# lmfaber/karma

Hardware: AMD Instinct MI355X
Metric: contigs+reads/sec for k-mer vec + shared-read graph build; HBM GB/s vs roofline (higher is better)
Workload: dtype u32 keys / i64 counts / f64 div

## Files before the change

### __graft_entry__.py

```python

import os
import subprocess
import sys

REPO = os.path.dirname(os.path.abspath(__file__))


def build() -> None:
    jobs = str(min(16, os.cpu_count() or 4))
    subprocess.run(["make", "-C", os.path.join(REPO, "karma_amd", "csrc"), "-j", jobs], check=True)
    subprocess.run(["make", "-C", os.path.join(REPO, "karma_amd", "csrc"), "fake_rccl"], check=True)
    subprocess.run(["make", "-C", os.path.join(REPO, "oracle")], check=True)
    sys.path.insert(0, REPO)
    import karma_amd
    from karma_amd import _lib

    _lib.load()


def smoke() -> None:
    from collections import OrderedDict

    import numpy as np

    sys.path.insert(0, REPO)
    from karma_amd import engine
    from oracle import oracle

    blob, offs, key_len = engine.synth_contigs(5, 300, 50, 900, 64)
    seqs = OrderedDict((f">ctg{i}", bytes(blob[offs[i]:offs[i + 1]]).decode()) for i in range(300))
    prof, cols, _ = engine.kmer_profile(seqs, "5p6")
    oprof, ocols, _ = oracle.calc_kmer_profile(seqs, "5p6")
    assert cols == ocols, "column set differs from the oracle"
    assert np.array_equal(prof.view(np.uint64), oprof.view(np.uint64)), "profile differs from the oracle"

    rec = engine.synth_records(5, 300, 0, 20000, True)
    e = engine.graph_from_records(rec, 300)
    r = rec.astype(np.int64)
    starts = np.flatnonzero(np.r_[True, r[1:, 0] != r[:-1, 0]])
    o = oracle.graph_groups(np.r_[starts, len(r)], r[:, 1], None, None, 300, dedup=True)
    assert np.array_equal(e.a, o["a"]) and np.array_equal(e.b, o["b"]), "edge set differs from the oracle"
    assert np.array_equal(e.weight.view(np.uint64), o["weight"].view(np.uint64)), "weights differ from the oracle"
    ef = engine.graph_from_records(engine.flag_records(rec), 300, flagged=True)
    assert np.array_equal(ef.a, o["a"]) and np.array_equal(ef.b, o["b"]), "flagged edge set differs from the oracle"
    assert np.array_equal(ef.weight.view(np.uint64), o["weight"].view(np.uint64)), "flagged weights differ"
    print(f"smoke ok: profile {prof.shape}, {len(e.a)} edges (pairs and flagged records), bit-exact vs oracle")


if __name__ == "__main__":
    build()
    if len(sys.argv) > 1 and sys.argv[1] == "smoke":
        smoke()
```

### karma_amd/csrc/graph_sets.hip

```cpp

#include <algorithm>
#include <cstdlib>
#include <cstring>
#include <memory>
#include <type_traits>

#include "karma_internal.h"

using namespace karma;

namespace {

#include "graph_device.h"

typedef unsigned int u32x4 __attribute__((ext_vector_type(4)));

constexpr int kMaxB = 2048;
constexpr int kMaxBc = 512;
constexpr int kNarrowB = 512, kNarrowBc = 128;
constexpr int kCrSmax = 64;
constexpr int kCrPieces = 512;
constexpr int kCgShift = 18;
constexpr int kOneGroupB = 128;
constexpr int kAppendMinBc = 129;
// ... 1438 lines not shown
                    pre += nibble_sum(w[i] & ((1u << bs) - 1u));
                    mine = (w[i] >> bs) & 15u;
                }
            }
            *beg = c * (int64_t)seg_cap * (kBinQ / 8) + pre;
            *len = mine;
            list_back(c, bucket < 32 ? h2.x : h2.y);
        },
        add8, nullptr, slots);
    __syncthreads();
    uint32_t* const wt = reinterpret_cast<uint32_t*>(slots) + wave * 64;
    auto stream8 = [&](uint64_t m, uint32_t seg) {
        const int n = __popcll(m);
        wave_lds_order();
        if (in_mask(m)) wt[rank_below(m)] = seg;
        wave_lds_order();
        u32x4 v[8];
#pragma unroll
        for (int t = 0; t < 8; ++t) {
            const int j = 8 * t + (lane >> 3);
            if (8 * t < n && j < n) v[t] = *reinterpret_cast<const u32x4*>(segs + (int64_t)wt[j] * kBinQ + 8 * (lane & 7));
        }
#pragma unroll
        for (int t = 0; t < 8; ++t)
            if (8 * t < n && 8 * t + (lane >> 3) < n) add8(v[t]);
    };
    const uint8_t bb = (uint8_t)bucket;
    const uint32_t nl = nlist;
    const bool listed = nl <= list_cap;
    const int64_t n_items = listed ? (int64_t)nl : c_hi - c_lo;
    for (int64_t i0 = (int64_t)wave * 64; i0 < n_items; i0 += kCRT) {
        const int64_t i = i0 + lane;
        const int64_t c = i < n_items ? c_lo + (listed ? (int64_t)blist[i] : i) : c_hi;
        uint4 h1 = {0u, 0u, 0u, 0u}, h2 = {0u, 0u, 0u, 0u}, h3 = {0u, 0u, 0u, 0u};
        if (c < c_hi) {
            h2 = hdr[kBinHdr * c + 2];
            h1 = hdr[kBinHdr * c + 1];
            h3 = hdr[kBinHdr * c + 3];
        }
        const uint64_t bm = h2.x | (uint64_t)h2.y << 32;
        uint64_t mb = lanes((bm >> bucket) & 1ull);
        if (!mb) continue;
        const uint32_t nb = h1.w;
        const uint32_t d[4] = {h2.z, h2.w, h3.x, h3.y};
        uint32_t hit = 0;
#pragma unroll
        for (int k = 0; k < 16; ++k)
            hit |= (((d[k >> 2] >> (8 * (k & 3))) & 0xFFu) == bb && (uint32_t)k < nb) ? 1u << k : 0u;
        for (uint32_t base = 0;;) {
            for (;;) {
                const uint64_t mm = lanes(in_mask(mb) && hit != 0u);
                if (!mm) break;
                uint32_t sg = 0;
                if (hit) {
                    const uint32_t k = (uint32_t)__builtin_ctz(hit);
                    hit &= hit - 1u;
                    sg = (uint32_t)c * seg_cap + seg_cap - 1u - (base + k);
                }
                stream8(mm, sg);
            }
            base += 16;
            mb &= lanes(base < nb);
            if (!mb) break;
            if (in_mask(mb)) {
                const u32x4 q = *reinterpret_cast<const u32x4*>(dir + c * (int64_t)dir_cap + base);
                const uint32_t e[4] = {q.x, q.y, q.z, q.w};
#pragma unroll
                for (int k = 0; k < 16; ++k)
                    hit |= (((e[k >> 2] >> (8 * (k & 3))) & 0xFFu) == bb && base + k < nb) ? 1u << k : 0u;
            }
        }
    }
    __syncthreads();
    uint32_t* out = part_ch + (int64_t)blockIdx.x * hn;
    for (int i = threadIdx.x; i < hn; i += kCRT) out[i] = h[slot(i)];
}

constexpr int kRT = 1024;
constexpr int kBand = 8192;
constexpr int kHashR = 4096;
constexpr int kHashF = 8192;
constexpr int kFT = 512;
constexpr int kSlotCap = kBand + kHashF;

template <int CAP, int THREADS>
struct HTab {
    uint32_t* keys;
    uint32_t* vals;
    int* nuniq;
    __device__ void init() {
        for (int t = threadIdx.x; t < CAP; t += THREADS) {
            keys[t] = kEmpty;
            vals[t] = 0;
        }
        if (threadIdx.x == 0) *nuniq = 0;
    }
    __device__ __forceinline__ bool insert(uint32_t key, uint32_t c) {
        uint32_t h = hash32(key) & (CAP - 1);
        for (int probe = 0; probe < CAP; ++probe) {
            const uint32_t k = __hip_atomic_load(&keys[h], __ATOMIC_RELAXED, __HIP_MEMORY_SCOPE_WORKGROUP);
            if (k == key) {
                atomicAdd(&vals[h], c);
                return true;
            }
            if (k == kEmpty) {
                const uint32_t old = atomicCAS(&keys[h], kEmpty, key);
                if (old == kEmpty || old == key) {
                    if (old == kEmpty) atomicAdd(nuniq, 1);
                    atomicAdd(&vals[h], c);
                    return true;
                }
            }
            h = (h + 1) & (CAP - 1);
        }
        return false;
    }
    __device__ int compact(int* cnt) {
        if (threadIdx.x == 0) *cnt = 0;
        __syncthreads();
        uint32_t my_k[CAP / THREADS], my_v[CAP / THREADS];
#pragma unroll
        for (int u = 0; u < CAP / THREADS; ++u) {
            my_k[u] = keys[u * THREADS + threadIdx.x];
            my_v[u] = vals[u * THREADS + threadIdx.x];
        }
        __syncthreads();
#pragma unroll
        for (int u = 0; u < CAP / THREADS; ++u) {
            if (my_k[u] != kEmpty) {
                const int pos = atomicAdd(cnt, 1);
                keys[pos] = my_k[u];
                vals[pos] = my_v[u];
            }
        }
        __syncthreads();
        return *cnt;
    }
};

__global__ void __launch_bounds__(kRT) pair_reduce_kernel(const uint32_t* __restrict__ pent, RunDir dir,
                                                          int n_pg, int bw, int bbits, int dbits, int B,
                                                          uint32_t* __restrict__ part_band,
                                                          uint32_t* __restrict__ part_keys,
                                                          uint32_t* __restrict__ part_cnt, int* __restrict__ part_n,
                                                          uint8_t* __restrict__ overflow) {
    __shared__ uint32_t band[kBand];
    __shared__ uint32_t hkeys[kHashR];
    __shared__ uint32_t hvals[kHashR];
    __shared__ int nuniq, cnt, ovf;
    __shared__ int slots[kRT];
    HTab<kHashR, kRT> t{hkeys, hvals, &nuniq};
    const int bucket = blockIdx.x / n_pg, grp = blockIdx.x % n_pg;
    const int band_n = dbits >= 0 ? (1 << (bw + dbits)) : 0;
    const uint32_t D = dbits >= 0 ? (1u << dbits) : 0u;
    int64_t f_lo, f_hi;
    group_range(dir.n, n_pg, grp, &f_lo, &f_hi);
    const int64_t sl = blockIdx.x;
    if (f_lo >= f_hi) {
        if (threadIdx.x == 0) part_n[sl] = -1;
        return;
    }
    t.init();
    for (int i = threadIdx.x; i < band_n; i += kRT) band[i] = 0;
    if (threadIdx.x == 0) ovf = 0;
    __syncthreads();
    const uint32_t bmask = (1u << bbits) - 1u, abase = (uint32_t)bucket << bw;
    auto add = [&](uint32_t e) {
        if (e == kEmpty) return;
        const uint32_t al = e >> bbits, d = (e & bmask) - (abase + al);
        if (d < D)
            __hip_atomic_fetch_add(&band[(al << dbits) | d], 1u, __ATOMIC_RELAXED, __HIP_MEMORY_SCOPE_WORKGROUP);
        else if (!t.insert(e, 1u))
            ovf = 1;
    };
    stream_runs(
        reinterpret_cast<const u32x4*>(pent), f_lo, f_hi, kRT,
        [&](int64_t f, int64_t* beg, uint32_t* len) {
            const uint32_t* o = dir.off + f * (B + 1) + bucket;
            *beg = (dir.base[f] + o[0]) >> 2;
            *len = (o[1] - o[0]) >> 2;
        },
        [&](const u32x4 v) {
            add(v.x), add(v.y), add(v.z), add(v.w);
            if (nuniq > kHashR - kHashR / 8) ovf = 1;
        },
        &ovf, slots);
    __syncthreads();
    if (ovf) {
        if (threadIdx.x == 0) overflow[bucket] = 1;
        return;
    }
    uint32_t* pb = part_band + sl * (int64_t)kBand;
    for (int i = threadIdx.x; i < band_n; i += kRT) pb[i] = band[i];
    const int n = t.compact(&cnt);
    uint32_t* pk = part_keys + sl * (int64_t)kHashR;
    uint32_t* pc = part_cnt + sl * (int64_t)kHashR;
    for (int i = threadIdx.x; i < n; i += kRT) {
        pk[i] = hkeys[i];
        pc[i] = hvals[i];
    }
    if (threadIdx.x == 0) part_n[sl] = n;
}

__device__ __forceinline__ uint32_t code_count(const uint32_t* __restrict__ part_ch, int n_cg, int bwc, int gi) {
    const int bc = gi >> (bwc + 3), i = gi & ((8 << bwc) - 1);
    const int hn = 8 << bwc;
    uint32_t k = 0;
    for (int g = 0; g < n_cg; ++g) k += part_ch[((int64_t)bc * n_cg + g) * hn + i];
    return k;
}

constexpr int kMaxSplit = 65;
struct SplitArgs {
    int n;
    int64_t b[kMaxSplit];
    int64_t* out;
};

template <int HF>
__global__ void __launch_bounds__(kFT) final_kernel(
    int n_pg, int n_cg, int bw, int bbits, int dbits, int bwc, const uint32_t* __restrict__ part_band,
    const uint32_t* __restrict__ part_ch, const uint32_t* __restrict__ part_keys,
    const uint32_t* __restrict__ part_cnt, const int* __restrict__ part_n, uint64_t* __restrict__ out_keys,
    int64_t* __restrict__ out_counts, int64_t* __restrict__ out_n, uint8_t* __restrict__ overflow, SplitArgs split,
    uint64_t* __restrict__ lb, int64_t* __restrict__ out_off) {
    __shared__ uint32_t bsum[kBand];
    __shared__ uint32_t rowpos[(kBand >> 3) + 1];
    __shared__ uint32_t hkeys[HF];
    __shared__ uint32_t hvals[HF];
    __shared__ uint32_t wsum[kFT / 64];
    __shared__ int nuniq, cnt;
    __shared__ int64_t base;
    const int bucket = blockIdx.x;
    auto skip = [&]() {
        if (threadIdx.x < 64) {
            const int64_t o = lookback_offset(lb, bucket, 0, (int)threadIdx.x);
            if (threadIdx.x == 0) {
                out_off[bucket] = o;
                out_n[bucket] = 0;
                if (bucket == (int)gridDim.x - 1) out_off[bucket + 1] = o;
            }
        }
    };
    if (overflow[bucket]) {
        skip();
        return;
    }
    HTab<HF, kFT> t{hkeys, hvals, &nuniq};
    const int band_n = dbits >= 0 ? (1 << (bw + dbits)) : 0;
    constexpr bool one_list = HF == kHashR;
    if (!one_list) t.init();
    for (int i = threadIdx.x; i < band_n; i += kFT) {
        uint32_t v = 0;
        for (int gi = 0; gi < n_pg; ++gi) {
            const int64_t sl = (int64_t)bucket * n_pg + gi;
            if (part_n[sl] >= 0) v += part_band[sl * kBand + i];
        }
        bsum[i] = v;
    }
    __syncthreads();
    if (n_cg > 0) {
        const int hn = 8 << bwc;
        for (int m0l = (bucket > 0 ? -3 : 0) + (int)threadIdx.x; m0l < (1 << bw); m0l += kFT) {
            const int64_t gi = ((int64_t)bucket << (bw + 3)) + 8 * (int64_t)m0l;
            const uint4* src = reinterpret_cast<const uint4*>(part_ch + (gi >> (bwc + 3)) * n_cg * hn + (gi & (hn - 1)));
            uint32_t k[8] = {};
            for (int g = 0; g < n_cg; ++g) {
                const uint4 a = src[(int64_t)g * (hn >> 2)], b = src[(int64_t)g * (hn >> 2) + 1];
                k[0] += a.x, k[1] += a.y, k[2] += a.z, k[3] += a.w;
                k[4] += b.x, k[5] += b.y, k[6] += b.z, k[7] += b.w;
            }
#pragma unroll
            for (int i1 = 0; i1 < 4; ++i1) {
                if (m0l + i1 < 0 || m0l + i1 >= (1 << bw)) continue;
#pragma unroll
                for (int j1 = i1; j1 < 4; ++j1) {
                    uint32_t acc = 0;
#pragma unroll
                    for (int M = 0; M < 8; ++M) {
                        const uint32_t bits = 1u | (uint32_t)M << 1;
                        if ((bits >> i1 & 1u) && (bits >> j1 & 1u)) acc += k[M];
                    }
                    if (acc) atomicAdd(&bsum[(m0l + i1) << dbits | (j1 - i1)], acc);
                }
            }
        }
        __syncthreads();
    }
    int nh;
    if (one_list) {
        nh = max(0, part_n[bucket]);
        for (int i = threadIdx.x; i < nh; i += kFT) {
            hkeys[i] = part_keys[(int64_t)bucket * kHashR + i];
            hvals[i] = part_cnt[(int64_t)bucket * kHashR + i];
        }
        __syncthreads();
    } else {
        for (int gi = 0; gi < n_pg; ++gi) {
            const int64_t sl = (int64_t)bucket * n_pg + gi;
            const int n = part_n[sl];
            bool full = false;
            for (int i = threadIdx.x; i < n; i += kFT)
                full |= !t.insert(part_keys[sl * kHashR + i], part_cnt[sl * kHashR + i]);
            if (__syncthreads_or(full)) {
                if (threadIdx.x == 0) overflow[bucket] = 1;
                skip();
                return;
            }
        }
        nh = t.compact(&cnt);
    }
    int p2 = 1;
    while (p2 < nh) p2 <<= 1;
    for (int i = nh + threadIdx.x; i < p2; i += kFT) {
        hkeys[i] = kEmpty;
// ... 633 lines not shown
                        KARMA_LAUNCH(ctx, "graph_classify",
                                     (classify2_kernel<decltype(ap)::value, true, decltype(rl)::value,
                                                       decltype(bn)::value, decltype(fl)::value>),
                                     cg, kCW, 0, C, Bn);
                        return KARMA_OK;
                    });
                };
                return bin ? go(std::false_type{}, std::true_type{})
                           : append ? go(std::true_type{}, std::false_type{}) : go(std::false_type{}, std::false_type{});
            });
        };
        if (probe) {
            KARMA_LAUNCH(ctx, "relabel_probe", relabel_probe_kernel, 1, kRelabelProbes, 0, rec, A, (uint32_t)N,
                         counters + 3, reinterpret_cast<uint64_t*>(cb), (int64_t)(ctrl_words + 2 * n_pblk + B));
            C.skip = counters + 3;
        } else if (fresh_ext) {
            C.skip = counters + 3;
            C.vote = counters + 4;
        }
        KARMA_TRY(classify(0, n_chunks));
    }
    KARMA_TRY(mark(1));
    if (A == 0) {
        KARMA_HIP(hipMemsetAsync(n_codes.ptr, 0, n_chunks * 4, ctx->stream));
        KARMA_HIP(hipMemsetAsync(n_gen.ptr, 0, n_chunks * 4, ctx->stream));
        if (bin) KARMA_HIP(hipMemsetAsync(bhdr.ptr, 0, n_chunks * 16 * kBinHdr, ctx->stream));
    }
    const RunDir cdir{cf_base.ptr, cf_off.ptr, counters + 1, blk_items};
    pdir = RunDir{pf_base.ptr, pf_off.ptr, counters + 2, blk_items + n_pblk};
    hipStream_t const main_stream = ctx->stream;
    const bool fork = fork_on() && !opts.single_stream && !(ctx->timing && ctx->timing_only.empty());
    hipStream_t fork_s = main_stream;
    if (fork) {
        KARMA_TRY(ctx_fork(ctx, !opts.fork));
        fork_s = opts.fork ? opts.fork : ctx->fork_stream;
        KARMA_HIP(hipEventRecord(ctx->fork_a, main_stream));
        KARMA_HIP(hipStreamWaitEvent(fork_s, ctx->fork_a, 0));
    }
    {
        StreamScope on_fork(ctx, fork_s);
        KARMA_LAUNCH(ctx, "graph_general", general_kernel, general_grid(ctx, n_chunks), kGW, 0, rec, A, (uint32_t)N,
                     codes.ptr, n_gen.ptr, n_chunks, plist.ptr, pcap, n_pl.ptr, blk_items + n_pblk, lpb, flags,
                     relabeled ? (const uint32_t*)remap_map.ptr : nullptr, (const unsigned*)(counters + 3), chunk);
        if (wide_p)
            KARMA_LAUNCH(ctx, "graph_pair_partition", partition_kernel<PairStreamWide>, n_pblk, kPT, 0, plist.ptr,
                         pcap, n_pl.ptr, n_chunks, lpb, g, pent.ptr, pdir);
        else
            KARMA_LAUNCH(ctx, "graph_pair_partition", partition_kernel<PairStream>, n_pblk, kPT, 0, plist.ptr, pcap,
                         n_pl.ptr, n_chunks, lpb, g, pent.ptr, pdir);
        KARMA_LAUNCH(ctx, "graph_pair_reduce", pair_reduce_kernel, nsl, kRT, 0, pent.ptr, pdir, n_pg, g.bw, g.bbits,
                     g.dbits, B, part_b.ptr, part_k.ptr, part_c.ptr, part_n.ptr, ovf);
        if (fork) KARMA_HIP(hipEventRecord(ctx->fork_b, fork_s));
    }
    if (bin) {
        KARMA_LAUNCH(ctx, "graph_code_reduce", code_seg_reduce_kernel, (int64_t)g.Bc * n_cg, kCRT, 0, bsegs.ptr,
                     reinterpret_cast<const uint4*>(bhdr.ptr), bdir.ptr, n_chunks, seg_cap, dir_cap, g.bwc, n_cg,
                     part_ch.ptr, back_list_cap(), slotted ? 1 : 0);
        KARMA_TRY(mark(2));
    } else if (g.Bc > 0) {
        uint16_t* const trash = cent.ptr + (ccap + 7) / 8 * 8;
        if (append && wide_c)
            KARMA_LAUNCH(ctx, "graph_code_partition", code_append_kernel<kMaxBc>, n_pblk, kPT, 0, codes.ptr, chunk,
                         n_codes.ptr, n_chunks, lpb, g, blk_hist.ptr, cent.ptr, trash, cdir, flags + 3);
        else if (append)
            KARMA_LAUNCH(ctx, "graph_code_partition", code_append_kernel<kNarrowBc>, n_pblk, kPT, 0, codes.ptr,
                         chunk, n_codes.ptr, n_chunks, lpb, g, blk_hist.ptr, cent.ptr, trash, cdir, flags + 3);
        else if (wide_c)
            KARMA_LAUNCH(ctx, "graph_code_partition", partition_kernel<CodeStreamWide>, n_pblk, kPT, 0, codes.ptr,
                         chunk, n_codes.ptr, n_chunks, lpb, g, cent.ptr, cdir);
        else
            KARMA_LAUNCH(ctx, "graph_code_partition", partition_kernel<CodeStream>, n_pblk, kPT, 0, codes.ptr, chunk,
                         n_codes.ptr, n_chunks, lpb, g, cent.ptr, cdir);
        KARMA_TRY(mark(2));
        KARMA_LAUNCH(ctx, "graph_code_reduce", code_reduce_kernel, (int64_t)g.Bc * n_cg, kCRT, 0, cent.ptr, cdir,
                     g.Bc, g.bwc, n_cg, part_ch.ptr);
    }
    KARMA_TRY(mark(4));
    if (fork) KARMA_HIP(hipStreamWaitEvent(main_stream, ctx->fork_b, 0));
    SplitArgs sa{};
    sa.n = (int)split_b.size();
    for (int r = 0; r < sa.n; ++r) sa.b[r] = split_b[r];
    sa.out = split_loc;
    if (n_pg == 1)
        KARMA_LAUNCH(ctx, "graph_bucket_final", final_kernel<kHashR>, B, kFT, 0, n_pg, n_cg, g.bw, g.bbits, g.dbits,
                     g.bwc, part_b.ptr, part_ch.ptr, part_k.ptr, part_c.ptr, part_n.ptr, slot_k.ptr, slot_c.ptr, n_per,
                     ovf, sa, lb, dst);
    else
        KARMA_LAUNCH(ctx, "graph_bucket_final", final_kernel<kHashF>, B, kFT, 0, n_pg, n_cg, g.bw, g.bbits, g.dbits,
                     g.bwc, part_b.ptr, part_ch.ptr, part_k.ptr, part_c.ptr, part_n.ptr, slot_k.ptr, slot_c.ptr, n_per,
                     ovf, sa, lb, dst);
    KARMA_TRY(mark(5));
    if (!deferred)
        KARMA_HIP(hipMemcpyAsync(const_cast<int64_t*>(hctrl), cb, ctrl_words * 8, hipMemcpyDeviceToHost,
                                 ctx->stream));
    return KARMA_OK;
}

int SetsJob::relabel() {
    const uint32_t n = (uint32_t)N;
    DevArray<uint32_t> rep, root;
    DevArray<unsigned> fill;
    DevArray<int64_t> size, base;
    KARMA_TRY(remap_map.alloc(ctx, N));
    KARMA_TRY(remap_inv.alloc(ctx, N));
    KARMA_TRY(rep.alloc(ctx, N));
    KARMA_TRY(root.alloc(ctx, N));
    KARMA_TRY(fill.alloc(ctx, N));
    KARMA_TRY(size.alloc(ctx, N + 1));
    KARMA_TRY(base.alloc(ctx, N + 1));
    KARMA_LAUNCH(ctx, "relabel_iota", iota_u32_kernel, grid_n(N), 256, 0, rep.ptr, N);
    const int64_t As = std::min<int64_t>(A, std::max<int64_t>(A / 32, int64_t(1) << 22));
    if (As) KARMA_LAUNCH(ctx, "relabel_hook", relabel_hook_kernel, grid_n(As), 256, 0, rec, As, n, rep.ptr);
    KARMA_HIP(hipMemsetAsync(size.ptr, 0, (N + 1) * 8, ctx->stream));
    KARMA_HIP(hipMemsetAsync(fill.ptr, 0, N * 4, ctx->stream));
    KARMA_LAUNCH(ctx, "relabel_root", relabel_root_kernel, grid_n(N + 1), 256, 0, rep.ptr, n, root.ptr, size.ptr);
    KARMA_TRY(scan_excl_i64(ctx, size.ptr, base.ptr, N + 1));
    KARMA_LAUNCH(ctx, "relabel_assign", relabel_assign_kernel, grid_n(N), 256, 0, root.ptr, base.ptr, n, fill.ptr,
                 remap_map.ptr, remap_inv.ptr);
    return KARMA_OK;
}

int SetsJob::finish(karma_pairs* out) {
    unsigned hc[4] = {0, 0, 0, 0};
    std::vector<uint8_t> hovf(B);
    int64_t U = 0;
    for (;;) {
        KARMA_HIP(hipStreamSynchronize(ctx->stream));
        const int* hf = reinterpret_cast<const int*>(hctrl);
        std::memcpy(hc, hctrl + 2, sizeof hc);
        std::memcpy(hovf.data(), hctrl + 6 + 2 * (B + 1), B);
        U = hctrl[6 + (B + 1) + B];
        KARMA_CHECK(!hf[0], KARMA_ERR_UNSORTED, "records are not grouped by read (read ids decrease)");
        KARMA_CHECK(!hf[1], KARMA_ERR_ARG, "a record's contig index is >= n_contigs (%lld)", (long long)N);
        KARMA_CHECK(!hf[3], KARMA_ERR_STATE, "code partition: block counts disagree with the classify histogram");
        if (!relabeled && hc[3]) {
            KARMA_TRY(relabel());
            relabeled = true;
            KARMA_TRY(launch());
            continue;
        }
        if (!hf[2]) break;
        KARMA_CHECK(attempt == 0, KARMA_ERR_STATE, "pair list capacity exceeded twice");
        attempt = 1;
        pcap = chunk * 9 / 2;
        KARMA_TRY(launch());
    }
    const unsigned n_big = hc[0];
    if (std::getenv("KARMA_DEBUG_GEN")) {
        std::vector<uint32_t> hg(n_chunks);
        KARMA_HIP(hipMemcpy(hg.data(), n_gen.ptr, n_chunks * 4, hipMemcpyDeviceToHost));
        uint64_t tot = 0;
        for (uint32_t x : hg) tot += x;
        std::fprintf(stderr, "[karma] general reads %llu, big reads %u, pair flushes %u\n", (unsigned long long)tot,
                     n_big, hc[2]);
    }
    DevArray<const uint64_t*> pk;
    DevArray<const int64_t*> pc;
    DevArray<int64_t> src_off;
    std::vector<std::unique_ptr<DevArray<uint64_t>>> keep_k;
    std::vector<std::unique_ptr<DevArray<int64_t>>> keep_c;
    const int64_t widen_threads = std::max<int64_t>(hc[2], (int64_t(8) << g.bw) + 24);
    bool any_ovf = false;
    for (int b = 0; b < B; ++b) {
        if (!hovf[b]) continue;
        if (!any_ovf) {
            KARMA_TRY(pk.alloc(ctx, B));
            KARMA_TRY(pc.alloc(ctx, B));
            KARMA_TRY(src_off.alloc(ctx, B));
            KARMA_HIP(hipMemcpyAsync(src_off.ptr, dst, B * 8, hipMemcpyDeviceToDevice, ctx->stream));
            KARMA_HIP(hipMemsetAsync(pk.ptr, 0, B * sizeof(void*), ctx->stream));
            KARMA_HIP(hipMemsetAsync(pc.ptr, 0, B * sizeof(void*), ctx->stream));
        }
        any_ovf = true;
// ... 152 lines not shown
```

### karma_amd/csrc/kmer.hip

```cpp

#include <algorithm>
#include <cstring>
#include <memory>

#include "karma_internal.h"

using namespace karma;

struct karma_contigs {
    karma_ctx* ctx = nullptr;
    int64_t n = 0, total = 0, words = 0, exc_bases = 0;
    int64_t zero_key_maxlen = -1;
    int64_t max_len = 0;
    DevArray<uint8_t> raw_own;
    DevArray<int64_t> off_own;
    DevArray<int32_t> keylen_own;
    const uint8_t* raw = nullptr;
    const int64_t* off = nullptr;
    const int32_t* keylen = nullptr;
    DevArray<int64_t> woff;
    DevArray<uint32_t> packed;
    DevArray<uint16_t> mask;
    DevArray<uint8_t> has_exc;
    DevArray<uint32_t> exc_list;
// ... 522 lines not shown
                }
            }
        }
        wave_lds_sync();
    }
}

template <bool C16>
__device__ __forceinline__ void write_row_wave(double* __restrict__ row, uint32_t* __restrict__ counts, int64_t M,
                                               int32_t klen, int* __restrict__ err, double* __restrict__ lut,
                                               int lane) {
    const double len = (double)klen;
    lut[lane] = lane ? (double)lane / len : 0.0;
    wave_lds_sync();
    auto val = [&](uint32_t a) {
        double v = lut[min(a, 63u)];
        if (a >= 64u) v = (double)a / len;
        return v;
    };
    if ((reinterpret_cast<uintptr_t>(row) & 15) == 0) {
        const int64_t M2 = M >> 1;
        for (int64_t j = lane; j < M2; j += 64) {
            uint32_t a, b;
            if (C16) {
                const uint32_t ab = counts[j];
                counts[j] = 0;
                a = ab & 0xFFFFu;
                b = ab >> 16;
            } else {
                const uint2 ab = reinterpret_cast<uint2*>(counts)[j];
                reinterpret_cast<uint2*>(counts)[j] = make_uint2(0u, 0u);
                a = ab.x;
                b = ab.y;
            }
            if ((a | b) && klen == 0) *err = 1;
            d2 v;
            v.x = val(a);
            v.y = val(b);
            typedef unsigned int u32x4_t __attribute__((ext_vector_type(4)));
            const uint64_t u = (uint64_t)row;
            const __amdgpu_buffer_rsrc_t rr = __builtin_amdgcn_make_buffer_rsrc(
                reinterpret_cast<void*>(((uint64_t)(uint32_t)__builtin_amdgcn_readfirstlane((int)(u >> 32)) << 32) |
                                        (uint32_t)__builtin_amdgcn_readfirstlane((int)(uint32_t)u)),
                0, (int)(M * 8), 0x00020000);
            const u32x4_t w = {(uint32_t)__double2loint(v.x), (uint32_t)__double2hiint(v.x),
                               (uint32_t)__double2loint(v.y), (uint32_t)__double2hiint(v.y)};
            __builtin_amdgcn_raw_buffer_store_b128(w, rr, (int)(j * 16), 0, kRowAux);
        }
        if ((M & 1) && lane == 0) {
            const uint32_t a = C16 ? counts[M >> 1] & 0xFFFFu : counts[M - 1];
            counts[C16 ? M >> 1 : M - 1] = 0;
            if (a && klen == 0) *err = 1;
            row_store(val(a), row + M - 1);
        }
    } else {
        uint16_t* c16 = reinterpret_cast<uint16_t*>(counts);
        for (int64_t j = lane; j < M; j += 64) {
            const uint32_t a = C16 ? c16[j] : counts[j];
            if (C16) c16[j] = 0;
            else counts[j] = 0;
            if (a && klen == 0) *err = 1;
            row_store(val(a), row + j);
        }
    }
}

__device__ __forceinline__ unsigned wave_total(unsigned x) {
    x += (unsigned)__builtin_amdgcn_update_dpp(0, (int)x, 0x111, 0xF, 0xF, false);
    x += (unsigned)__builtin_amdgcn_update_dpp(0, (int)x, 0x112, 0xF, 0xF, false);
    x += (unsigned)__builtin_amdgcn_update_dpp(0, (int)x, 0x114, 0xF, 0xF, false);
    x += (unsigned)__builtin_amdgcn_update_dpp(0, (int)x, 0x118, 0xF, 0xF, false);
    x += (unsigned)__builtin_amdgcn_update_dpp(0, (int)x, 0x142, 0xA, 0xF, false);
    x += (unsigned)__builtin_amdgcn_update_dpp(0, (int)x, 0x143, 0xC, 0xF, false);
    return (unsigned)__builtin_amdgcn_readlane((int)x, 63);
}

__host__ __device__ constexpr int64_t hist_words(int64_t M, bool c16) {
    return c16 ? (((M + 1) >> 1) + 3) & ~int64_t(3) : (M + 3) & ~int64_t(3);
}
__host__ __device__ constexpr int64_t tab_entries(bool p56, uint32_t S) { return p56 ? 1088 : (int64_t)S; }

constexpr int kProfWaves = 6;
template <bool P56, bool C16>
__global__ void __launch_bounds__(kPBlock) __attribute__((amdgpu_waves_per_eu(kProfWaves, kProfWaves)))
profile_wave_kernel(
    const uint32_t* __restrict__ packed, const uint16_t* __restrict__ mask, const uint8_t* __restrict__ has_exc,
    const int64_t* __restrict__ woff, const int64_t* __restrict__ off, const uint8_t* __restrict__ raw,
    const int32_t* __restrict__ keylen, int64_t n, int k, bool with_len, const int32_t* __restrict__ col_of_ord,
    const uint64_t* __restrict__ exc, int64_t X, const int32_t* __restrict__ col_of_exc, int64_t M,
    double* __restrict__ out, int64_t ld, int* __restrict__ err, int S, int64_t* __restrict__ row_tot,
    int64_t exc0, const int64_t* __restrict__ m_dev) {
    extern __shared__ __attribute__((aligned(16))) uint32_t lds[];
    const int wave = __builtin_amdgcn_readfirstlane(threadIdx.x >> 6), lane = threadIdx.x & 63, wpb = blockDim.x >> 6;
    uint16_t* tab = reinterpret_cast<uint16_t*>(lds);
    const int t_pad = (int)((tab_entries(P56, S) + 7) & ~7);
    const int h_words = (int)hist_words(M, C16);
    if (m_dev) {
        M = *m_dev;
        ld = M;
    }
    uint32_t* counts = lds + t_pad / 2 + wave * (h_words + kProfWin);
    uint32_t* win = counts + h_words;
    uint16_t* mbuf = reinterpret_cast<uint16_t*>(win + 80);
    double* lut = reinterpret_cast<double*>(win);
    if (P56) {
        for (int o = threadIdx.x; o < 1088; o += blockDim.x) {
            uint32_t ord;
            if (o < 1024) {
                ord = 5u * o;
            } else {
                const uint32_t h3 = o - 1024, c6 = h3 << 6 | rev3(h3);
                ord = (c6 >> 2) * 5u + 1u + (c6 & 3u);
            }
            tab[o] = (uint16_t)col_of_ord[ord];
        }
    } else {
        for (int o = threadIdx.x; o < S; o += blockDim.x) tab[o] = (uint16_t)col_of_ord[o];
    }
    for (int j = lane; j < h_words; j += 64) counts[j] = 0;
    __syncthreads();
    const int kmin = P56 ? 5 : k;
    struct Meta {
        int64_t s = 0, L = 0, w0 = 0;
        int32_t klen = 0;
        bool exc = false;
    };
    auto meta = [&](int64_t cc, Meta& m) {
        if (cc < n) {
            m.s = off[cc];
            m.L = off[cc + 1] - m.s;
            m.w0 = woff[cc];
            m.klen = keylen[cc];
            const int64_t ce = exc0 + cc;
            const uint32_t hw = reinterpret_cast<const uint32_t*>(has_exc)[ce >> 2];
            m.exc = ((hw >> (8 * (ce & 3))) & 0xFFu) != 0;
        }
    };
    const int64_t stride = (int64_t)gridDim.x * wpb;
    int64_t c = (int64_t)blockIdx.x * wpb + wave;
    Meta cur, nxt;
    Stage st0;
    meta(c, cur);
    if (c < n) st0.load(packed, mask, cur.exc, cur.w0, lane);
    for (; c < n; c += stride) {
        meta(c + stride, nxt);
        const int64_t L = cur.L;
        unsigned my = 0;
        if (!cur.exc) {
            count_clean<P56, C16>(st0, packed, cur.w0, L, kmin, k, tab, counts, win, lane, my);
        } else {
            const uint8_t* craw = raw + cur.s;
            auto add = [&](uint32_t cl) {
                hist_add<C16>(counts, cl);
                ++my;
            };
            for_each_window(packed, mask, true, cur.w0, L - kmin + 1, win, mbuf, lane,
                            [&](int64_t i, const Window& v) {
                if (P56) {
                    if (v.clean(5)) add(tab[v.code(5)]);
                    else add(col_of_exc[lower_bound_u64(exc, X, key_from_bytes(craw + i, 5, true))]);
                    if (i + 6 <= L) {
                        if (v.clean(6)) {
                            const uint32_t c6 = v.code(6);
                            if (pal6_code(c6)) add(tab[1024u + (c6 >> 6)]);
                        } else if (pal_bytes(craw + i, 6)) {
                            add(col_of_exc[lower_bound_u64(exc, X, key_from_bytes(craw + i, 6, true))]);
                        }
// ... 551 lines not shown
```

### karma_amd/csrc/step.hip

```cpp
#include <algorithm>
#include <chrono>
#include <cstdlib>
#include <cstring>
#include <deque>
#include <memory>
#include <thread>
#include <vector>

#include "karma_internal.h"

using namespace karma;

namespace {

constexpr int kRing = 64;
constexpr int kLag = 3;

struct StepStatus {
    uint64_t seq;
    int64_t slow;
    int64_t err;
    int64_t U;
    int64_t E;
    int64_t pad[3];
};
static_assert(sizeof(StepStatus) == 64, "status entry");

constexpr int kET = 512;
constexpr int kMaxRuns = 64;

__device__ __forceinline__ bool is_head(const uint64_t* __restrict__ k, int64_t i, uint64_t key) {
    return i == 0 || k[i - 1] != key;
}
__device__ __forceinline__ int64_t run_sum(const uint64_t* __restrict__ k, const int64_t* __restrict__ c, int64_t n,
                                           int64_t i, uint64_t key) {
    int64_t s = c[i];
    for (int64_t j = i + 1; j < n && k[j] == key; ++j) s += c[j];
    return s;
}

__global__ void __launch_bounds__(kET) step_edge_count_kernel(const uint64_t* __restrict__ keys,
                                                              const int64_t* __restrict__ counts,
                                                              const int64_t* __restrict__ n_dev, int64_t n_tot,
                                                              int64_t* __restrict__ totals,
                                                              int64_t* __restrict__ tile_cnt,
                                                              int64_t* __restrict__ st) {
    const int64_t n = *n_dev;
    if (blockIdx.x == 0 && threadIdx.x < 3) st[threadIdx.x] = 0;
    const int64_t stride = (int64_t)gridDim.x * kET, gid = (int64_t)blockIdx.x * kET + threadIdx.x;
    const int64_t a_first = n ? (int64_t)(keys[0] >> 32) : n_tot;
    const int64_t a_last = n ? (int64_t)(keys[n - 1] >> 32) : n_tot;
    for (int64_t c = gid; c < min(a_first, n_tot); c += stride) totals[c] = 0;
    for (int64_t c = a_last + 1 + gid; c < n_tot; c += stride) totals[c] = 0;
    const int64_t tiles = (n + kET - 1) / kET;
    for (int64_t t = blockIdx.x; t < tiles; t += gridDim.x) {
        const int64_t i = t * kET + threadIdx.x;
        bool f = false;
        if (i < n) {
            const uint64_t k = keys[i];
            const uint32_t a = (uint32_t)(k >> 32), b = (uint32_t)k;
            if (i > 0) {
                const uint32_t pa = (uint32_t)(keys[i - 1] >> 32);
                const uint32_t lim = (int64_t)a < n_tot ? a : (uint32_t)n_tot;
                for (uint32_t c = pa + 1; c < lim; ++c) totals[c] = 0;
                if ((int64_t)a < n_tot && pa != a && a != b) totals[a] = 0;
            } else if ((int64_t)a < n_tot && a != b) {
                totals[a] = 0;
            }
            if (is_head(keys, i, k) && (int64_t)b < n_tot) {
                const int64_t s = run_sum(keys, counts, n, i, k);
                if (a == b) totals[a] = s;
                else f = s != 0;
            }
        }
        const int cnt = __syncthreads_count(f);
        if (threadIdx.x == 0) tile_cnt[t] = cnt;
    }
}

__global__ void __launch_bounds__(kET) step_edge_write_kernel(
    const uint64_t* __restrict__ keys, const int64_t* __restrict__ counts, const int64_t* __restrict__ n_dev,
    const int64_t* __restrict__ totals, const int64_t* __restrict__ tile_cnt, uint32_t* __restrict__ ea,
    uint32_t* __restrict__ eb, int64_t* __restrict__ es, double* __restrict__ ew, int64_t* __restrict__ st,
    int64_t n_tot) {
    __shared__ int64_t wsum[kET / 64];
    __shared__ int64_t base_s;
    const int64_t n = *n_dev;
    const int64_t tiles = (n + kET - 1) / kET;
    const int lane = threadIdx.x & 63, wave = threadIdx.x >> 6;
    if (blockIdx.x == 0 && tiles == 0 && threadIdx.x == 0) st[2] = 0;
    for (int64_t t = blockIdx.x; t < tiles; t += gridDim.x) {
        int64_t b = 0;
        for (int64_t j = threadIdx.x; j < t; j += kET) b += tile_cnt[j];
#pragma unroll
        for (int d = 32; d >= 1; d >>= 1) b += __shfl_xor(b, d, 64);
        if (lane == 0) wsum[wave] = b;
        __syncthreads();
        if (threadIdx.x == 0) {
            int64_t s = 0;
            for (int w = 0; w < kET / 64; ++w) s += wsum[w];
            base_s = s;
        }
        const int64_t i = t * kET + threadIdx.x;
        uint64_t k = 0;
        int64_t c = 0;
        bool f = false;
        if (i < n) {
            k = keys[i];
            const uint32_t a = (uint32_t)(k >> 32), bb = (uint32_t)k;
            if ((int64_t)bb >= n_tot) {
                st[1] = 1;
            } else if (a != bb && is_head(keys, i, k)) {
                c = run_sum(keys, counts, n, i, k);
                f = c != 0;
            }
        }
        const uint64_t m = __ballot(f);
        __syncthreads();
        if (lane == 0) wsum[wave] = __popcll(m);
        __syncthreads();
        int64_t before = 0, total = 0;
        for (int w = 0; w < kET / 64; ++w) {
            if (w < wave) before += wsum[w];
            total += wsum[w];
        }
        const int64_t base = base_s;
        if (t == tiles - 1 && threadIdx.x == 0) st[2] = base + total;
        if (f) {
            const int64_t o = base + before + __popcll(m & ((1ull << lane) - 1ull));
            const uint32_t a = (uint32_t)(k >> 32), bb = (uint32_t)k;
            const int64_t ta = totals[a], tb = totals[bb];
            ea[o] = a;
            eb[o] = bb;
            es[o] = c;
            if (ta == 0 || tb == 0) {
                st[0] = 1;
                ew[o] = 0.0;
            } else {
                const double x = __ddiv_rn((double)c, (double)ta);
                const double y = __ddiv_rn((double)c, (double)tb);
                ew[o] = __dadd_rn(x, y) * 0.5;
            }
        }
        __syncthreads();
    }
}

constexpr int kMarkOne = 2;
constexpr int kMarkTwo = 4;
constexpr int kMarkOneFlagged = 2;
constexpr int64_t kAltMaxRecords = int64_t(1) << 27;
constexpr int kMT = 1024;
constexpr int kMLds = 8192;
constexpr int kMFast = 8;
constexpr int kMG = 16;
struct RunSrc {
    int nr, B, bw;
    int64_t b[kMaxRuns + 1];
    int64_t slot = 0;
    int64_t* n_out = nullptr;
};

__device__ __forceinline__ int64_t count_below(const uint64_t* __restrict__ a, int64_t lo, int64_t hi, uint64_t k,
                                               bool le) {
    int64_t n = hi - lo, base = lo;
    while (n > 0) {
        const int64_t half = n >> 1;
        const uint64_t m = a[base + half];
        const bool before = le ? m <= k : m < k;
        base = before ? base + half + 1 : base;
        n = before ? n - half - 1 : half;
    }
    return base;
}

__global__ void __launch_bounds__(256) step_merge_kernel(const uint64_t* __restrict__ keys,
                                                         const int64_t* __restrict__ counts,
                                                         const int64_t* __restrict__ dst,
                                                         const int64_t* __restrict__ split_loc, RunSrc rs,
                                                         uint64_t* __restrict__ ko, int64_t* __restrict__ co,
                                                         int64_t* __restrict__ bad) {
    __shared__ int64_t ro[kMaxRuns + 1], re[kMaxRuns + 1], rt[kMaxRuns + 1];
    __shared__ int64_t wlo[kMaxRuns], whi[kMaxRuns];
    __shared__ int wbase[kMaxRuns];
    __shared__ int all_fit;
    __shared__ uint64_t wkeys[kMLds];
    const int nr = rs.nr;
    const int64_t U = rs.slot > 0 ? 0 : dst[rs.B];
    if (rs.slot == 0 && threadIdx.x <= (unsigned)nr) {
        const int64_t bd = rs.b[threadIdx.x];
        const int64_t b = bd >> rs.bw;
        ro[threadIdx.x] = bd <= 0 ? 0 : (b < rs.B ? dst[b] + split_loc[threadIdx.x] : U);
    }
    __syncthreads();
    if (threadIdx.x < (unsigned)nr) {
        const int r = threadIdx.x;
        if (rs.slot > 0) {
            const uint64_t h = keys[(int64_t)r * rs.slot];
            if (h >> 62) {
                atomicOr(reinterpret_cast<unsigned long long*>(bad), (h >> 63 ? 2ull : 0ull) | (h >> 62 & 1 ? 4ull : 0ull));
            }
            ro[r] = (int64_t)r * rs.slot + 1;
            re[r] = ro[r] + (int64_t)min<uint64_t>(h & ~(3ull << 62), (uint64_t)(rs.slot - 1));
        } else {
            re[r] = ro[r + 1];
        }
    }
    __syncthreads();
    if (rs.n_out && blockIdx.x == 0 && threadIdx.x == 0) {
        int64_t tot = 0;
        for (int r = 0; r < nr; ++r) tot += re[r] - ro[r];
        *rs.n_out = tot;
    }
    if (threadIdx.x == 0) {
        int64_t t = 0;
        for (int r = 0; r < nr; ++r) {
            rt[r] = t;
            t += (re[r] - ro[r] + kMT - 1) / kMT;
        }
        rt[nr] = t;
    }
    __syncthreads();
    const int64_t tiles = rt[nr];
    const int lane = threadIdx.x & 63, g = lane & (kMG - 1), grp = threadIdx.x / kMG;
    const unsigned long long gmask = ((1ull << kMG) - 1ull) << (lane & ~(kMG - 1));
    for (int64_t tile = blockIdx.x; tile < tiles; tile += gridDim.x) {
        int r = 0;
        while (r + 1 < nr && rt[r + 1] <= tile) ++r;
        const int64_t t0 = ro[r] + (tile - rt[r]) * kMT, t1 = min(re[r], t0 + kMT);
        for (int q0 = 0; q0 < 2 * nr; q0 += 256 / kMG) {
            const int q = q0 + grp;
            const int sr = q >> 1;
            const bool search = q < 2 * nr && sr != r;
            int64_t lo = search ? ro[sr] : 0, hi = search ? re[sr] : 0;
            const uint64_t k = search ? keys[(q & 1) ? t1 - 1 : t0] : 0;
            const bool le = sr < r;
            if (hi > lo) {
                const uint64_t f = keys[lo], l = keys[hi - 1];
                if (le ? l <= k : l < k) lo = hi;
                else if (le ? f > k : f >= k) hi = lo;
            }
            for (;;) {
                const bool more = hi - lo > kMG;
                if (!__ballot(more)) break;
                const int64_t step = (hi - lo + kMG - 1) / kMG;
                const int64_t p = min(hi - 1, lo + (int64_t)(g + 1) * step - 1);
                const bool before = more && (le ? keys[p] <= k : keys[p] < k);
                const int c = __popcll(__ballot(before) & gmask);
                if (more) {
                    const int64_t nlo = c ? min(hi, lo + (int64_t)c * step) : lo;
                    const int64_t nhi = c < kMG ? min(hi, lo + (int64_t)(c + 1) * step - 1) : hi;
                    lo = nlo;
                    hi = nhi;
                }
            }
            const int64_t p = lo + g;
            const bool before = p < hi && (le ? keys[p] <= k : keys[p] < k);
            const int64_t ans = lo + __popcll(__ballot(before) & gmask);
            if (search && g == 0) {
                if (q & 1) whi[sr] = ans;
                else wlo[sr] = ans;
            }
        }
        __syncthreads();
        if (threadIdx.x == 0) {
            int used = 0, fit = 1;
            for (int sr = 0; sr < nr; ++sr) {
                if (sr == r) continue;
                if (whi[sr] < wlo[sr]) whi[sr] = wlo[sr];
// ... 665 lines not shown
        }
        karma_kmer_plan* plan = nullptr;
        rc = kmer_plan_create(ctx, store, s->kmode, po, &plan);
        if (!rc && s->world > 1) {
            if (xs_on && s->one_comm) {
                rc = stream_after(&s->ev_pres, side, xs);
                if (!rc && s->sync_set) {
                    rc = stream_after(&s->ev_sync, s->main_s, xs);
                    s->sync_set = false;
                }
                {
                    StreamScope on_xs(ctx, xs);
                    if (!rc) rc = exchange_presence(s, plan, s->comm);
                    if (!rc) rc = stream_after(&s->ev_pres2, xs, side);
                }
            } else {
                rc = exchange_presence(s, plan, s->scomm ? s->scomm : s->comm);
            }
        }
        int64_t* const m_dev = s->m_ring.ptr + seq % kRing;
        if (!rc) rc = kmer_finalize_device(plan, m_dev, s->mring_d + seq % kRing);
        if (rc && !sequential && pz.ptr) (void)hipMemsetAsync(pz.ptr, 0, pz.n * 4, side);
        if (!rc) rc = ensure_prof(s, tl.prof, (size_t)std::max<int64_t>(1, s->n_loc * kmer_m_cap(plan)));
        if (!rc && ctx->mark_set && !sequential) {
            if (counted_call("hipStreamWaitEvent")) ++t_hip_calls;
            rc = hipStreamWaitEvent(side, ctx->mark_ev, 0) == hipSuccess ? KARMA_OK : KARMA_ERR_HIP;
        }
        if (!rc && s->n_loc) rc = kmer_profile_device_m(plan, tl.prof.ptr, m_dev);
        if (plan) karma_kmer_plan_destroy(plan);
    }
    KARMA_TRY(rc);
    if (xs_on) {
        KARMA_TRY(stream_after(&s->ev_rec, ms, xs));
        if (s->sync_set) {
            KARMA_TRY(stream_after(&s->ev_sync, s->main_s, xs));
            s->sync_set = false;
        }
    }
    StreamScope on_tail(ctx, xs_on ? xs : ms);
    const uint64_t* lk = v.keys;
    const int64_t* lc = v.counts;
    const int64_t* n_dev = v.dst + v.B;
    int64_t* mbad = nullptr;
    const int cu = ctx->cu_count;
    int64_t cap = v.cap;
    if (s->exchange) {
        if (!tl.mbad.ptr) {
            KARMA_TRY(tl.mbad.alloc(ctx, 1));
            KARMA_HIP(hipMemsetAsync(tl.mbad.ptr, 0, 8, ctx->stream));
        }
        RunSrc rs{};
        rs.nr = s->nranks;
        rs.B = v.B;
        rs.bw = v.bw;
        for (int r = 0; r <= s->nranks; ++r) rs.b[r] = s->bounds[r];
        KARMA_CHECK((int)v.split_b.size() == s->nranks + 1, KARMA_ERR_STATE, "karma_step: the split hint was lost");
        const uint64_t* mkeys = v.keys;
        const int64_t* mcounts = v.counts;
        if (s->world > 1) {
            const int W = s->world;
            const int64_t slot = s->kc + 1;
            KARMA_TRY(ensure_arr(ctx, tl.sk, W * slot));
            KARMA_TRY(ensure_arr(ctx, tl.sc, W * slot));
            KARMA_TRY(ensure_arr(ctx, tl.rk, W * slot));
            KARMA_TRY(ensure_arr(ctx, tl.rc, W * slot));
            KARMA_TRY(ensure_arr(ctx, tl.nm, 1));
            KARMA_LAUNCH(ctx, "exchange_pack", step_pack_kernel,
                         (int)std::max<int64_t>(1, std::min<int64_t>((v.cap + 255) / 256, 4 * cu)), 256, 0, v.keys,
                         v.counts, v.dst, v.split_loc, rs, slot, tl.sk.ptr, tl.sc.ptr, v.flags, v.counters, v.ovf);
            std::vector<int64_t> off(W + 1);
            for (int r = 0; r <= W; ++r) off[r] = (int64_t)r * slot * 8;
            KARMA_TRY(karma_comm_alltoallv_kv(s->comm, tl.sk.ptr, tl.sc.ptr, off.data(), tl.rk.ptr, tl.rc.ptr,
                                              off.data()));
            rs.slot = slot;
            rs.n_out = tl.nm.ptr;
            mkeys = tl.rk.ptr;
            mcounts = tl.rc.ptr;
            cap = W * (slot - 1);
            n_dev = tl.nm.ptr;
        }
        KARMA_TRY(ensure_arr(ctx, tl.mk, cap));
        KARMA_TRY(ensure_arr(ctx, tl.mc, cap));
        const int64_t tiles_cap = (cap + kMT - 1) / kMT + s->nranks;
        KARMA_LAUNCH(ctx, "merge_rank", step_merge_kernel, (int)std::min<int64_t>(tiles_cap, 8 * cu), 256, 0, mkeys,
                     mcounts, v.dst, v.split_loc, rs, tl.mk.ptr, tl.mc.ptr, tl.mbad.ptr);
        lk = tl.mk.ptr;
        lc = tl.mc.ptr;
        mbad = tl.mbad.ptr;
    }
    KARMA_TRY(ensure_arr(ctx, tl.tot, s->n_glob));
    KARMA_TRY(ensure_arr(ctx, tl.tile_cnt, (cap + kET - 1) / kET + 1));
    KARMA_TRY(ensure_arr(ctx, tl.est, 3));
    KARMA_TRY(ensure_arr(ctx, tl.ea, cap));
    KARMA_TRY(ensure_arr(ctx, tl.eb, cap));
    KARMA_TRY(ensure_arr(ctx, tl.es, cap));
    KARMA_TRY(ensure_arr(ctx, tl.ew, cap));
    const int grid = (int)std::max<int64_t>(1, std::min<int64_t>((cap + kET - 1) / kET, 4 * cu));
    KARMA_LAUNCH(ctx, "edge_count", step_edge_count_kernel, grid, kET, 0, lk, lc, n_dev, s->n_glob, tl.tot.ptr,
                 tl.tile_cnt.ptr, tl.est.ptr);
    if (s->world > 1) KARMA_TRY(allgather_slices(s, tl.tot.ptr));
    KARMA_LAUNCH(ctx, "edge_weights", step_edge_write_kernel, grid, kET, 0, lk, lc, n_dev, tl.tot.ptr,
                 tl.tile_cnt.ptr, tl.ea.ptr, tl.eb.ptr, tl.es.ptr, tl.ew.ptr, tl.est.ptr, s->n_glob);
    KARMA_CHECK(seq != s->fault_seq, KARMA_ERR_STATE, "karma_step: injected fault in deferred step %llu",
                (unsigned long long)seq);
    KARMA_LAUNCH(ctx, "step_status", step_status_kernel, 1, 256, 0, v.flags, v.counters, v.ovf, v.B, v.dst, mbad,
                 tl.est.ptr, s->ring_d + seq % kRing, seq, v.ctrl, v.ctrl ? v.ctrl_need : (int64_t)0);
    if (xs_on) {
        if (!s->ev_tail[par]) KARMA_HIP(hipEventCreateWithFlags(&s->ev_tail[par], hipEventDisableTiming));
        if (counted_call("hipEventRecord")) ++t_hip_calls;
        KARMA_HIP(hipEventRecord(s->ev_tail[par], xs));
        s->tail_set[par] = true;
        s->tail_last = par;
    }
    fail.armed = false;
    s->pending.push_back({seq, store, rec, A, flg});
    return KARMA_OK;
}

}

extern "C" {

int karma_step_create(karma_ctx* ctx, karma_comm* comm, karma_comm* side_comm, int kmode, int64_t n_glob,
                      const int64_t* bounds, int nranks, int rank, karma_step** out) {
    KARMA_TRY(ctx_begin(ctx));
    KARMA_CHECK(out && bounds && nranks >= 1 && nranks <= kMaxRuns && rank >= 0 && rank < nranks && n_glob >= 1,
                KARMA_ERR_ARG, "karma_step_create: bad arguments (nranks %d, rank %d)", nranks, rank);
    int world = 1, crank = 0;
    if (comm) KARMA_TRY(karma_comm_info(comm, &world, &crank));
    KARMA_CHECK(world == 1 || (world == nranks && crank == rank), KARMA_ERR_ARG,
                "karma_step_create: communicator of %d ranks (rank %d) for %d owners (rank %d)", world, crank,
                nranks, rank);
    KARMA_CHECK(nranks == 1 || (bounds[0] == 0 && bounds[nranks] == n_glob), KARMA_ERR_ARG,
                "owner bounds must span [0, n_glob)");
    KARMA_CHECK(bounds[0] >= 0 && bounds[nranks] <= n_glob, KARMA_ERR_ARG, "owner bounds outside [0, n_glob)");
    for (int r = 0; r < nranks; ++r)
        KARMA_CHECK(bounds[r] <= bounds[r + 1], KARMA_ERR_ARG, "owner bounds must not decrease");
    std::unique_ptr<karma_step> s(new karma_step());
    s->ctx = ctx;
    s->comm = world > 1 ? comm : nullptr;
    s->scomm = world > 1 && side_comm != comm ? side_comm : nullptr;
    s->one_comm = s->scomm == nullptr;
    s->kmode = kmode;
    s->world = world;
    s->rank = rank;
    s->nranks = nranks;
    s->emulate = world == 1 && nranks > 1 ? nranks : 0;
    if (const char* e = getenv("KARMA_STEP_STREAMS")) s->streams = atoi(e) == 1 ? 1 : atoi(e) == 2 ? 2 : 0;
    if (const char* e = getenv("KARMA_STEP_DEFER_RANKS")) s->defer_ranks = atoi(e) != 0;
    if (const char* e = getenv("KARMA_STEP_XSTREAM")) s->xstream = atoi(e) != 0;
    if (const char* e = getenv("KARMA_STEP_STALL_S")) s->stall_s = std::max(1, atoi(e));
    if (const char* e = getenv("KARMA_STEP_LAG")) s->lag = std::max(1, std::min(kRing / 2, atoi(e)));
    if (const char* e = getenv("KARMA_STEP_FAULT_SEQ")) s->fault_seq = strtoull(e, nullptr, 10);
    s->n_glob = n_glob;
    s->bounds.assign(bounds, bounds + nranks + 1);
    s->c_lo = bounds[rank];
    s->n_loc = bounds[rank + 1] - bounds[rank];
    s->exchange = nranks > 1;
    int lo = 0, hi = 0;
    KARMA_HIP(hipDeviceGetStreamPriorityRange(&lo, &hi));
    KARMA_HIP(hipStreamCreateWithPriority(&s->main_s, hipStreamNonBlocking, hi));
    KARMA_HIP(hipStreamCreateWithPriority(&s->alt_s, hipStreamNonBlocking, hi));
    KARMA_HIP(hipStreamCreateWithPriority(&s->side_s, hipStreamNonBlocking, 0));
    KARMA_HIP(hipStreamCreateWithPriority(&s->side_alt_s, hipStreamNonBlocking, 0));
    void *hm = nullptr, *dm = nullptr;
    KARMA_HIP(hipHostMalloc(&s->ring_mem, kRing * sizeof(StepStatus) + kRing * 8,
                            hipHostMallocMapped | hipHostMallocCoherent));
    hm = s->ring_mem;
    KARMA_HIP(hipHostGetDevicePointer(&dm, hm, 0));
    s->mring_h = reinterpret_cast<int64_t*>(static_cast<uint8_t*>(hm) + kRing * sizeof(StepStatus));
    s->mring_d = reinterpret_cast<int64_t*>(static_cast<uint8_t*>(dm) + kRing * sizeof(StepStatus));
    KARMA_HIP(hipHostMalloc(reinterpret_cast<void**>(&s->graves_h), kRing * 4 * 8, hipHostMallocDefault));
    {
        StreamScope on_main(ctx, s->main_s);
        KARMA_TRY(s->m_ring.alloc(ctx, kRing));
    }
    s->ring_h = static_cast<StepStatus*>(hm);
    s->ring_d = static_cast<StepStatus*>(dm);
    std::memset(hm, 0, kRing * sizeof(StepStatus) + kRing * 8);
    *out = s.release();
// ... 183 lines not shown
```

Baseline: 126.9 billion.

## Move kernel LDS to dynamic shared memory and retune edge/profile launch sizes

```diff
diff --git a/__graft_entry__.py b/__graft_entry__.py
--- a/__graft_entry__.py
+++ b/__graft_entry__.py
@@ -8,7 +8,7 @@
 
 def build() -> None:
     jobs = str(min(16, os.cpu_count() or 4))
-    subprocess.run(["make", "-C", os.path.join(REPO, "karma_amd", "csrc"), "-j", jobs], check=True)
+    subprocess.run(["make", "-C", os.path.join(REPO, "karma_amd", "csrc"), "-j", jobs, "all", "asm"], check=True)
     subprocess.run(["make", "-C", os.path.join(REPO, "karma_amd", "csrc"), "fake_rccl"], check=True)
     subprocess.run(["make", "-C", os.path.join(REPO, "oracle")], check=True)
     sys.path.insert(0, REPO)
diff --git a/karma_amd/csrc/graph_sets.hip b/karma_amd/csrc/graph_sets.hip
--- a/karma_amd/csrc/graph_sets.hip
+++ b/karma_amd/csrc/graph_sets.hip
@@ -1544,6 +1544,8 @@
 constexpr int kHashF = 8192;
 constexpr int kFT = 512;
 constexpr int kSlotCap = kBand + kHashF;
+constexpr int kFinalRowpos = ((kBand >> 3) + 1 + 3) & ~3;
+constexpr size_t final_lds_bytes(int hf) { return (size_t)(kBand + kFinalRowpos + 2 * hf + kFT / 64 + 2) * 4 + 8; }
 
 template <int CAP, int THREADS>
 struct HTab {
@@ -1686,13 +1688,15 @@
     const uint32_t* __restrict__ part_cnt, const int* __restrict__ part_n, uint64_t* __restrict__ out_keys,
     int64_t* __restrict__ out_counts, int64_t* __restrict__ out_n, uint8_t* __restrict__ overflow, SplitArgs split,
     uint64_t* __restrict__ lb, int64_t* __restrict__ out_off) {
-    __shared__ uint32_t bsum[kBand];
-    __shared__ uint32_t rowpos[(kBand >> 3) + 1];
-    __shared__ uint32_t hkeys[HF];
-    __shared__ uint32_t hvals[HF];
-    __shared__ uint32_t wsum[kFT / 64];
-    __shared__ int nuniq, cnt;
-    __shared__ int64_t base;
+    extern __shared__ __attribute__((aligned(16))) uint32_t final_lds[];
+    uint32_t* const bsum = final_lds;
+    uint32_t* const rowpos = bsum + kBand;
+    uint32_t* const hkeys = rowpos + kFinalRowpos;
+    uint32_t* const hvals = hkeys + HF;
+    uint32_t* const wsum = hvals + HF;
+    int& nuniq = *reinterpret_cast<int*>(wsum + kFT / 64);
+    int& cnt = *(&nuniq + 1);
+    int64_t& base = *reinterpret_cast<int64_t*>(&nuniq + 2);
     const int bucket = blockIdx.x;
     auto skip = [&]() {
         if (threadIdx.x < 64) {
@@ -2492,13 +2496,13 @@
     for (int r = 0; r < sa.n; ++r) sa.b[r] = split_b[r];
     sa.out = split_loc;
     if (n_pg == 1)
-        KARMA_LAUNCH(ctx, "graph_bucket_final", final_kernel<kHashR>, B, kFT, 0, n_pg, n_cg, g.bw, g.bbits, g.dbits,
-                     g.bwc, part_b.ptr, part_ch.ptr, part_k.ptr, part_c.ptr, part_n.ptr, slot_k.ptr, slot_c.ptr, n_per,
-                     ovf, sa, lb, dst);
+        KARMA_LAUNCH(ctx, "graph_bucket_final", final_kernel<kHashR>, B, kFT, final_lds_bytes(kHashR), n_pg, n_cg,
+                     g.bw, g.bbits, g.dbits, g.bwc, part_b.ptr, part_ch.ptr, part_k.ptr, part_c.ptr, part_n.ptr,
+                     slot_k.ptr, slot_c.ptr, n_per, ovf, sa, lb, dst);
     else
-        KARMA_LAUNCH(ctx, "graph_bucket_final", final_kernel<kHashF>, B, kFT, 0, n_pg, n_cg, g.bw, g.bbits, g.dbits,
-                     g.bwc, part_b.ptr, part_ch.ptr, part_k.ptr, part_c.ptr, part_n.ptr, slot_k.ptr, slot_c.ptr, n_per,
-                     ovf, sa, lb, dst);
+        KARMA_LAUNCH(ctx, "graph_bucket_final", final_kernel<kHashF>, B, kFT, final_lds_bytes(kHashF), n_pg, n_cg,
+                     g.bw, g.bbits, g.dbits, g.bwc, part_b.ptr, part_ch.ptr, part_k.ptr, part_c.ptr, part_n.ptr,
+                     slot_k.ptr, slot_c.ptr, n_per, ovf, sa, lb, dst);
     KARMA_TRY(mark(5));
     if (!deferred)
         KARMA_HIP(hipMemcpyAsync(const_cast<int64_t*>(hctrl), cb, ctrl_words * 8, hipMemcpyDeviceToHost,
diff --git a/karma_amd/csrc/kmer.hip b/karma_amd/csrc/kmer.hip
--- a/karma_amd/csrc/kmer.hip
+++ b/karma_amd/csrc/kmer.hip
@@ -628,7 +628,7 @@
 
 constexpr int kProfWaves = 6;
 template <bool P56, bool C16>
-__global__ void __launch_bounds__(kPBlock) __attribute__((amdgpu_waves_per_eu(kProfWaves, kProfWaves)))
+__global__ void __launch_bounds__(kPBlock) __attribute__((amdgpu_waves_per_eu(kProfWaves, kProfWaves + 1)))
 profile_wave_kernel(
     const uint32_t* __restrict__ packed, const uint16_t* __restrict__ mask, const uint8_t* __restrict__ has_exc,
     const int64_t* __restrict__ woff, const int64_t* __restrict__ off, const uint8_t* __restrict__ raw,
diff --git a/karma_amd/csrc/step.hip b/karma_amd/csrc/step.hip
--- a/karma_amd/csrc/step.hip
+++ b/karma_amd/csrc/step.hip
@@ -26,7 +26,7 @@
 };
 static_assert(sizeof(StepStatus) == 64, "status entry");
 
-constexpr int kET = 512;
+constexpr int kET = 256;
 constexpr int kMaxRuns = 64;
 
 __device__ __forceinline__ bool is_head(const uint64_t* __restrict__ k, int64_t i, uint64_t key) {
@@ -184,7 +184,7 @@
     __shared__ int64_t wlo[kMaxRuns], whi[kMaxRuns];
     __shared__ int wbase[kMaxRuns];
     __shared__ int all_fit;
-    __shared__ uint64_t wkeys[kMLds];
+    extern __shared__ __attribute__((aligned(16))) uint64_t wkeys[];
     const int nr = rs.nr;
     const int64_t U = rs.slot > 0 ? 0 : dst[rs.B];
     if (rs.slot == 0 && threadIdx.x <= (unsigned)nr) {
@@ -1016,7 +1016,8 @@
         KARMA_TRY(ensure_arr(ctx, tl.mk, cap));
         KARMA_TRY(ensure_arr(ctx, tl.mc, cap));
         const int64_t tiles_cap = (cap + kMT - 1) / kMT + s->nranks;
-        KARMA_LAUNCH(ctx, "merge_rank", step_merge_kernel, (int)std::min<int64_t>(tiles_cap, 8 * cu), 256, 0, mkeys,
+        KARMA_LAUNCH(ctx, "merge_rank", step_merge_kernel, (int)std::min<int64_t>(tiles_cap, 8 * cu), 256,
+                     kMLds * sizeof(uint64_t), mkeys,
                      mcounts, v.dst, v.split_loc, rs, tl.mk.ptr, tl.mc.ptr, tl.mbad.ptr);
         lk = tl.mk.ptr;
         lc = tl.mc.ptr;
@@ -1029,7 +1030,7 @@
     KARMA_TRY(ensure_arr(ctx, tl.eb, cap));
     KARMA_TRY(ensure_arr(ctx, tl.es, cap));
     KARMA_TRY(ensure_arr(ctx, tl.ew, cap));
-    const int grid = (int)std::max<int64_t>(1, std::min<int64_t>((cap + kET - 1) / kET, 4 * cu));
+    const int grid = (int)std::max<int64_t>(1, std::min<int64_t>((cap + kET - 1) / kET, 8 * cu));
     KARMA_LAUNCH(ctx, "edge_count", step_edge_count_kernel, grid, kET, 0, lk, lc, n_dev, s->n_glob, tl.tot.ptr,
                  tl.tile_cnt.ptr, tl.est.ptr);
     if (s->world > 1) KARMA_TRY(allgather_slices(s, tl.tot.ptr));
```

Measured after the change: 126.9 billion (median of 2 runs). Within noise of the previous version (-0.0%).
